# DeepGraphLearning/ultra_torchdrug

Measured on AMD Instinct MI355X. Metric: edges aggregated/sec, FB15k237-shaped 6L x 64d rspmm Bellman-Ford (predict: the reference's 18 rspmm layers per batch as 6 relation-graph + 6 entity-graph launches, tails and heads in one pass), higher is better.
Workload: dtype f32

## Files before the change

ultra_torchdrug_amd/csrc/dense.inc:

```

namespace {

struct LinearParams {
    const float *input;
    const float *weight;
    const float *bias;
    float *out;
    long long rows;
    int relu;
};

template <int K, int N>
__global__ __launch_bounds__(kCbWaves * 64, 1) void linear_kernel(const LinearParams p) {
    static_assert(K == N && (K == 64 || K == 128), "supported shapes: 64x64, 128x128");
    constexpr int kStride = K + 4;
    constexpr int kOutTiles = N / 32;
    extern __shared__ __attribute__((aligned(16))) float dl_lds[];
    float *w_lds = dl_lds;
    const int lane = threadIdx.x & 63;
    const int wl = uniform(threadIdx.x >> 6);
    float *tile = dl_lds + N * kStride + wl * (32 * kStride);
    const int i = lane & 31, h = lane >> 5;
    for (int idx = threadIdx.x; idx < N * (K / 4); idx += kCbWaves * 64) {
        const int r = idx / (K / 4), c = (idx % (K / 4)) * 4;
// ... 334 lines not shown
int launch_linear(const LinearParams &p, int n_cu, hipStream_t stream) {
    constexpr int kStride = K + 4;
    const size_t lds = (size_t)(K * kStride + kCbWaves * 32 * kStride) * sizeof(float);
    const long long n_tiles = (p.rows + 31) / 32;
    long long blocks = (n_tiles + kCbWaves - 1) / kCbWaves;
    if (blocks > n_cu) blocks = n_cu;
    return launch_with_lds(linear_kernel<K, K>, p, (int)blocks, lds, stream, kCbWaves * 64, (int)lds);
}

}

namespace {

constexpr int kProjMaxLayers = 8;
struct ProjectParams {
    const float *relation;
    const float *w1[kProjMaxLayers], *b1[kProjMaxLayers], *w2[kProjMaxLayers], *b2[kProjMaxLayers];
    float *out[kProjMaxLayers];
    long long rows;
    int batch, n_rel, n_layers, blocks_per_layer;
    int repeat;
    long long stride_b, stride_r;
};

__global__ __launch_bounds__(kCbWaves * 64, 1) void project_kernel(const ProjectParams p) {
    constexpr int K = 64, kStride = K + 4;
    extern __shared__ __attribute__((aligned(16))) float pj_lds[];
    float *w1_lds = pj_lds, *w2_lds = pj_lds + K * kStride;
    const int lane = threadIdx.x & 63;
    const int wl = uniform(threadIdx.x >> 6);
    float *tile = pj_lds + 2 * K * kStride + wl * (32 * kStride);
    const int i = lane & 31, h = lane >> 5;
    const int l = blockIdx.x / p.blocks_per_layer, bl = blockIdx.x % p.blocks_per_layer;
    for (int idx = threadIdx.x; idx < K * (K / 4); idx += kCbWaves * 64) {
        const int r = idx / (K / 4), c = (idx % (K / 4)) * 4;
        *reinterpret_cast<f32x4 *>(w1_lds + r * kStride + c) = *reinterpret_cast<const f32x4 *>(p.w1[l] + r * K + c);
        *reinterpret_cast<f32x4 *>(w2_lds + r * kStride + c) = *reinterpret_cast<const f32x4 *>(p.w2[l] + r * K + c);
    }
    __syncthreads();
    const float bias1[2] = {p.b1[l][i], p.b1[l][i + 32]}, bias2[2] = {p.b2[l][i], p.b2[l][i + 32]};
    float *out = p.out[l];
    const long long n_tiles = (p.rows + 31) / 32;
    const long long wave_global = (long long)bl * kCbWaves + wl;
    const long long wave_total = (long long)p.blocks_per_layer * kCbWaves;
    auto gemm = [&](const float *w_lds, const float (&bias)[2], f32x16 (&acc)[2]) {
#pragma unroll
        for (int tt = 0; tt < 2; ++tt)
#pragma unroll
            for (int r = 0; r < 16; ++r) acc[tt][r] = bias[tt];
#pragma unroll
        for (int q = 0; q < K / 8; ++q) {
            const f32x4 av = *reinterpret_cast<const f32x4 *>(tile + i * kStride + (K / 2) * h + 4 * q);
#pragma unroll
            for (int tt = 0; tt < 2; ++tt) {
                const f32x4 wv = *reinterpret_cast<const f32x4 *>(w_lds + (i + 32 * tt) * kStride + (K / 2) * h + 4 * q);
                acc[tt] = __builtin_amdgcn_mfma_f32_32x32x2f32(av.x, wv.x, acc[tt], 0, 0, 0);
                acc[tt] = __builtin_amdgcn_mfma_f32_32x32x2f32(av.y, wv.y, acc[tt], 0, 0, 0);
                acc[tt] = __builtin_amdgcn_mfma_f32_32x32x2f32(av.z, wv.z, acc[tt], 0, 0, 0);
                acc[tt] = __builtin_amdgcn_mfma_f32_32x32x2f32(av.w, wv.w, acc[tt], 0, 0, 0);
            }
        }
        asm volatile("s_waitcnt lgkmcnt(0)" ::: "memory");
    };
    auto spill = [&](const f32x16 (&acc)[2], bool relu) {
#pragma unroll
        for (int tt = 0; tt < 2; ++tt)
#pragma unroll
            for (int r = 0; r < 16; ++r) {
                const int row = (r & 3) + 8 * (r >> 2) + 4 * h;
                float v = acc[tt][r];
                if (relu) v = !(v <= 0.0f) ? v : 0.0f;
                tile[row * kStride + 32 * tt + i] = v;
            }
        asm volatile("s_waitcnt lgkmcnt(0)" ::: "memory");
    };
    for (long long t = wave_global; t < n_tiles; t += wave_total) {
        const long long row0 = t * 32;
        const long long last = p.rows - 1;
#pragma unroll
        for (int q = 0; q < 8; ++q) {
            const int r = 4 * q + (lane >> 4), c = (lane & 15) * 4;
            long long gr = row0 + r;
            gr = gr < last ? gr : last;
            const long long b = gr / p.n_rel, rel = gr - b * p.n_rel;
            *reinterpret_cast<f32x4 *>(tile + r * kStride + c) = *reinterpret_cast<const f32x4 *>(p.relation + b * p.stride_b + rel * p.stride_r + c);
        }
        asm volatile("s_waitcnt vmcnt(0) lgkmcnt(0)" ::: "memory");
        f32x16 acc[2];
        gemm(w1_lds, bias1, acc);
        spill(acc, true);
        gemm(w2_lds, bias2, acc);
        spill(acc, false);
#pragma unroll
        for (int q = 0; q < 8; ++q) {
            const int r = 4 * q + (lane >> 4), c = (lane & 15) * 4;
            const long long gr = row0 + r;
            if (gr < p.rows) {
                const long long b = gr / p.n_rel, rel = gr % p.n_rel;
                const f32x4 v = *reinterpret_cast<const f32x4 *>(tile + r * kStride + c);
                for (int j = 0; j < p.repeat; ++j)
                    *reinterpret_cast<f32x4 *>(out + (rel * ((long long)p.batch * p.repeat) + b + (long long)j * p.batch) * K + c) = v;
            }
        }
        asm volatile("s_waitcnt lgkmcnt(0)" ::: "memory");
    }
}

__global__ __launch_bounds__(256) void filtered_rank_kernel(const float *pred, long long row_stride, long long n_cand,
                                                            const int64_t *target, const int32_t *filt_ptr,
                                                            const int32_t *filt_node, int64_t *rank) {
    __shared__ long long part[4];
    const long long q = blockIdx.x;
    const float *row = pred + q * row_stride;
    const float pos = row[target[q]];
    long long count = 0;
    for (long long c = threadIdx.x; c < n_cand; c += blockDim.x) count += (pos <= row[c]) ? 1 : 0;
    if (filt_ptr != nullptr) {
        const int lo = filt_ptr[q], hi = filt_ptr[q + 1];
        for (int k = lo + (int)threadIdx.x; k < hi; k += (int)blockDim.x) count -= (pos <= row[filt_node[k]]) ? 1 : 0;
    }
#pragma unroll
    for (int off = 32; off > 0; off >>= 1) count += __shfl_down(count, off, 64);
    if ((threadIdx.x & 63) == 0) part[threadIdx.x >> 6] = count;
    __syncthreads();
    if (threadIdx.x == 0) rank[q] = part[0] + part[1] + part[2] + part[3] + 1;
}

}

extern "C" {

// ... 109 lines not shown
```

ultra_torchdrug_amd/csrc/frontier.inc:

```

struct FrontierParams {
    const int32_t *src_ptr;
    const int32_t *dst;
    const int32_t *rel;
    const float *weight;
    const int32_t *fwd_rank;
    const float *relation;
    const int32_t *bnode;
    const float *bvec;
    float *out;
    long long F;
    int piece_len;
    int slices;
    int n_rel;
    int piece_shift;
    const int32_t *run_prefix;
    int32_t *row_list;
    const int32_t *list_offset;
    int list_len;
};

constexpr int kFrontierThreads = 256;
constexpr int kFrontierU = 4;

template <bool UNIT_W>
__global__ __launch_bounds__(kFrontierThreads) void frontier_kernel(const FrontierParams p) {
    const int lane = threadIdx.x & 63;
    const int b = blockIdx.x;
    const long long col = (long long)b * 64 + (lane & 15) * 4;
    const int groups_per_block = kFrontierThreads / 16;
    const int g = blockIdx.y * groups_per_block + (threadIdx.x >> 4);
    const int n_groups = p.slices * groups_per_block;
    const int h = p.bnode[b];
    const qf4 q = *reinterpret_cast<const qf4 *>(p.bvec + col);
    const int lo = p.src_ptr[h], hi = p.src_ptr[h + 1];

    if (g == 0) {
        bool self_loop = false;
        int a = lo, z = hi;
        while (a < z) {
            const int m = (a + z) >> 1;
            if (p.dst[m] < h) a = m + 1; else z = m;
        }
        self_loop = a < hi && p.dst[a] == h;
        if (!self_loop) {
            const qf4 zero = {0.0f, 0.0f, 0.0f, 0.0f};
            *reinterpret_cast<qf4 *>(p.out + (long long)h * p.F + col) = zero + q;
        }
        if (p.row_list != nullptr && (lane & 15) == 0 && p.list_offset[b + 1] - 1 < p.list_len)
            p.row_list[p.list_offset[b + 1] - 1] = self_loop ? -1 : h * (int)(p.F / 64) + b;
    }

// ... 75 lines not shown
        }
#pragma unroll
        for (int u = 0; u < kFrontierU; ++u) {
            if (done) break;
            const int eu = e + u;
            if (eu >= hi) { done = true; break; }
            if (d[u] != cur) {
                if (eu >= end) { done = true; break; }
                close_run();
                cur = d[u];
                run_first = eu;
                cur_piece = -1;
                have_total = false;
            }
            const int piece_of_edge = k[u] / p.piece_len;
            if (piece_of_edge != cur_piece) {
                close_piece();
                cur_piece = piece_of_edge;
                piece_end_rank = (cur_piece + 1) * p.piece_len;
                piece = qf4{0.0f, 0.0f, 0.0f, 0.0f};
            }
            qf4 y = rv[u] * q;
            if constexpr (!UNIT_W) y = w[u] * y;
            piece = piece + y;
        }
        e += kFrontierU;
    }
    close_run();
}

constexpr int kFrontierLdsThreads = 1024;
constexpr int kFrontierLdsSlices = 8;

template <bool UNIT_W>
__global__ __launch_bounds__(kFrontierLdsThreads) void frontier_lds_kernel(const FrontierParams p) {
    extern __shared__ __attribute__((aligned(16))) float fl_msg[];
    const int lane = threadIdx.x & 63;
    const int sub = lane & 15;
    const int n_query = (int)(p.F / 64);
    const int b = blockIdx.x % n_query;
    const int slice = blockIdx.x / n_query;
    const long long col = (long long)b * 64 + sub * 4;
    const int h = p.bnode[b];
    const qf4 q = *reinterpret_cast<const qf4 *>(p.bvec + col);
    {
        const float *rel_b = p.relation + (long long)b * 64;
        const float *q_b = p.bvec + (long long)b * 64;
        for (int i = threadIdx.x; i < p.n_rel * 16; i += kFrontierLdsThreads) {
            const int r = i >> 4, c4 = (i & 15) * 4;
            const qf4 rv = *reinterpret_cast<const qf4 *>(rel_b + (long long)r * p.F + c4);
            const qf4 qq = *reinterpret_cast<const qf4 *>(q_b + c4);
            reinterpret_cast<qf4 *>(fl_msg)[i] = rv * qq;
        }
    }
    __syncthreads();
    const qf4 *msg = reinterpret_cast<const qf4 *>(fl_msg) + sub;

    const int groups_per_block = kFrontierLdsThreads / 16;
    const int g = slice * groups_per_block + (threadIdx.x >> 4);
    const int n_groups = p.slices * groups_per_block;
    const int lo = p.src_ptr[h], hi = p.src_ptr[h + 1];

    const int list_base = p.row_list != nullptr ? p.list_offset[b] : 0;
    if (g == 0) {
        int a = lo, z = hi;
        while (a < z) {
            const int m = (a + z) >> 1;
            if (p.dst[m] < h) a = m + 1; else z = m;
        }
        const bool self_loop = a < hi && p.dst[a] == h;
        if (!self_loop) {
            const qf4 zero = {0.0f, 0.0f, 0.0f, 0.0f};
            *reinterpret_cast<qf4 *>(p.out + (long long)h * p.F + col) = zero + q;
        }
        if (p.row_list != nullptr && sub == 0 && p.list_offset[b + 1] - 1 < p.list_len)
            p.row_list[p.list_offset[b + 1] - 1] = self_loop ? -1 : h * n_query + b;
    }

    const int n = hi - lo;
    if (n <= 0) return;
    const int per = (n + n_groups - 1) / n_groups;
    int e = lo + g * per;
    const int end = min(e + per, hi);
    if (e >= end) return;
    if (e > lo) {
        const int prev = p.dst[e - 1];
        int a = e, step = 1;
        while (a < hi && p.dst[a] == prev) { a += step; step <<= 1; }
        if (a > e) {
            int z = min(a, hi);
            a = a - (step >> 1) + 1;
            while (a < z) {
                const int m = (a + z) >> 1;
                if (p.dst[m] == prev) a = m + 1; else z = m;
            }
        }
        e = a;
    }
    if (e >= end) return;

    int slot = 0;
    if (p.row_list != nullptr) slot = list_base + p.run_prefix[e] - p.run_prefix[lo];
    int cur = p.dst[e];
    int cur_piece = -1;
    bool open = false, have_total = false;
    qf4 total = {0.0f, 0.0f, 0.0f, 0.0f};
    qf4 piece = {0.0f, 0.0f, 0.0f, 0.0f};
    auto close_piece = [&]() {
        if (open) {
            total = have_total ? total + piece : (qf4{0.0f, 0.0f, 0.0f, 0.0f} + piece);
            have_total = true;
        }
    };
    auto close_run = [&](int dest) {
        close_piece();
        qf4 v = total;
        v = v + ((dest == h) ? q : qf4{0.0f, 0.0f, 0.0f, 0.0f});
        *reinterpret_cast<qf4 *>(p.out + (long long)dest * p.F + col) = v;
        if (p.row_list != nullptr) {
            if (sub == 0 && slot < p.list_len) p.row_list[slot] = dest * n_query + b;
            ++slot;
        }
    };
    auto load_ids = [&](int e0, int &d, int &r, int &k, float &w) {
        const int eu = min(e0 + sub, hi - 1);
        d = p.dst[eu];
        r = p.rel[eu];
        k = p.fwd_rank[eu];
        w = 1.0f;
        if constexpr (!UNIT_W) w = p.weight[eu];
    };
    const int bp = (lane & 48) * 4;
    const int grp_shift = (lane >> 4) * 16;
    auto from = [&](int u, int v) -> int { return __builtin_amdgcn_ds_bpermute(bp + 4 * u, v); };

    int nd, nr, nk;
    float nw;
    load_ids(e, nd, nr, nk, nw);
    bool done = false;
    while (!done) {
        const int md = nd, mr = nr, mk = nk;
        const float mw = nw;
        load_ids(e + 16, nd, nr, nk, nw);
        const int mp = p.piece_shift >= 0 ? (mk >> p.piece_shift) : (mk / p.piece_len);
        const int prev_d = __builtin_amdgcn_update_dpp(cur, md, 0x111, 0xf, 0xf, false);
        const int prev_p = __builtin_amdgcn_update_dpp(cur_piece, mp, 0x111, 0xf, 0xf, false);
        const int n_valid = min(16, hi - e);
        const bool starts_run = (md != prev_d) && sub < n_valid;
        const bool starts_piece = (starts_run || mp != prev_p) && sub < n_valid;
        const uint32_t run_bits = (uint32_t)(__builtin_amdgcn_ballot_w64(starts_run) >> grp_shift) & 0xffffu;
        const uint32_t piece_bits = (uint32_t)(__builtin_amdgcn_ballot_w64(starts_piece) >> grp_shift) & 0xffffu;
        const int room = end - e;
        const uint32_t beyond = room >= 16 ? 0u : (room <= 0 ? 0xffffu : (0xffffu << room) & 0xffffu);
        const uint32_t stop_bits = run_bits & beyond;
        const int n_sum = min(n_valid, stop_bits ? __builtin_ctz(stop_bits) : 16);
        done = n_sum < 16;
#pragma unroll
        for (int half = 0; half < 2; ++half) {
            qf4 y[8];
#pragma unroll
            for (int v = 0; v < 8; ++v) {
                const int u = 8 * half + v;
                y[v] = msg[from(u, mr) * 16];
                if constexpr (!UNIT_W) y[v] = __builtin_bit_cast(float, from(u, __builtin_bit_cast(int, mw))) * y[v];
            }
            const uint32_t any = (run_bits | piece_bits) >> (8 * half) & 0xffu;
            if (any == 0u && n_sum >= 8 * half + 8) {
#pragma unroll
                for (int v = 0; v < 8; ++v) piece = piece + y[v];
                continue;
            }
#pragma unroll
            for (int v = 0; v < 8; ++v) {
                const int u = 8 * half + v;
                if (u < n_sum) {
                    if ((run_bits >> u) & 1u) {
                        close_run(u == 0 ? cur : from(u - 1, md));
                        have_total = false;
                        open = false;
                    }
                    if ((piece_bits >> u) & 1u) {
                        close_piece();
                        open = true;
                        piece = qf4{0.0f, 0.0f, 0.0f, 0.0f};
                    }
                    piece = piece + y[v];
                }
            }
        }
        if (n_sum > 0) {
            cur = from(n_sum - 1, md);
            cur_piece = from(n_sum - 1, mp);
        }
        e += 16;
    }
    close_run(cur);
}

constexpr int kSparseMaxQueries = 128;
struct ConstFillParams {
    qf4 *out;
    long long n4;
    const float *bias, *gamma, *beta;
    float eps;
    int relu, shortcut;
    const int32_t *src_ptr, *run_prefix, *bnode;
    int n_query;
    int list_len;
    int32_t *list_offset;
};

__global__ __launch_bounds__(256) void const_fill_kernel(const ConstFillParams p) {
    __shared__ __attribute__((aligned(16))) float c[64];
    __shared__ int slots[kSparseMaxQueries];
    if (threadIdx.x < 64) {
        const int j = threadIdx.x;
        float v = p.bias[j];
        if (p.gamma != nullptr) {
            float s0 = 0.0f, s1 = 0.0f;
            for (int k = 0; k < 32; ++k) { s0 = s0 + p.bias[k]; s1 = s1 + p.bias[32 + k]; }
            const float mean = (s0 + s1) * (1.0f / 64.0f);
            float q0 = 0.0f, q1 = 0.0f;
            for (int k = 0; k < 32; ++k) {
                const float d0 = p.bias[k] - mean, d1 = p.bias[32 + k] - mean;
                q0 = q0 + d0 * d0;
                q1 = q1 + d1 * d1;
            }
            const float var = (q0 + q1) * (1.0f / 64.0f);
            const float inv = 1.0f / sqrtf(var + p.eps);
            v = ((v - mean) * inv) * p.gamma[j] + p.beta[j];
        }
        if (p.relu) v = !(v <= 0.0f) ? v : 0.0f;
        c[j] = p.shortcut ? v + 0.0f : v;
    }
    if (blockIdx.x == 0) {
        if ((int)threadIdx.x < p.n_query) {
            const int h = p.bnode[threadIdx.x];
            const int lo = p.src_ptr[h], hi = p.src_ptr[h + 1];
            slots[threadIdx.x] = (hi > lo ? p.run_prefix[hi - 1] - p.run_prefix[lo] + 1 : 0) + 1;
        }
        __syncthreads();
        if (threadIdx.x == 0) {
            int total = 0;
            for (int b = 0; b < p.n_query; ++b) {
                p.list_offset[b] = total;
                total += slots[b];
            }
            p.list_offset[p.n_query] = total;
        }
    }
    __syncthreads();
    const qf4 *c4 = reinterpret_cast<const qf4 *>(c);
    for (long long i = (long long)blockIdx.x * 256 + threadIdx.x; i < p.n4; i += (long long)gridDim.x * 256) p.out[i] = c4[i & 15];
}

__global__ __launch_bounds__(256) void zero_fill_kernel(qf4 *out, long long n4) {
    const qf4 zero = {0.0f, 0.0f, 0.0f, 0.0f};
    for (long long i = (long long)blockIdx.x * 256 + threadIdx.x; i < n4; i += (long long)gridDim.x * 256) out[i] = zero;
}

struct BoundaryRowsParams {
    const int32_t *src_ptr;
    const int32_t *dst;
    const int32_t *rel;
    const float *weight;
    const float *relation;
    const float *grad;
    const int32_t *bnode;
    float *partial;
    float *d_input;
    long long F;
};

// ... 64 lines not shown
```

ultra_torchdrug_amd/csrc/plan_path.h:

```cpp
#ifndef ULTRA_PLAN_PATH_H
#define ULTRA_PLAN_PATH_H

#include <cstddef>
#include <cstdint>

#include "ultra_rspmm.h"

namespace ultra_detail {

constexpr int kTile = 64;
constexpr int kXcd = 8;
constexpr int kMaxLdsBytes = 156 * 1024;
constexpr int kLdsHeader = 16;
constexpr int kPlanBlock = 1024;
constexpr int kPlanRgBlock = 512;

enum Kind { KIND_FWD = 0, KIND_DX = 1, KIND_DREL = 2 };
enum Family { FAM_DENSE = 0, FAM_ROWGROUP = 1, FAM_QUAD = 2, FAM_PACKED = 3, FAM_GENERAL = 4 };
enum RelMode { REL_L2 = 0, REL_LDS = 1, REL_PART = 2 };
enum ActMode { ACT_NONE = 0, ACT_BITS = 2, ACT_NODE = 3 };
enum UnrollClass { UNROLL_U = 0, UNROLL_UW = 1, UNROLL_UX = 2 };
enum Fixup { FIX_NONE = 0, FIX_PLAIN = 1, FIX_MANY = 2 };

struct Knobs {
    bool force_general = false;
    bool no_x_lds = false;
    bool no_quad = false;
    bool no_rowgroup = false;
    bool wide_groups = false;
    bool no_concurrent_tiles = false;
    bool no_dense = false;
    bool no_dead_words = false;
    bool no_paired = false;
    bool force_paired = false;
    bool score_lds_rows = false;
    bool combine_lds_rows = false;
};

inline Knobs decode_knobs(int mask) {
    Knobs k;
    k.force_general = (mask & 1) != 0;
    k.no_x_lds = (mask & 2) != 0;
    k.no_quad = (mask & 4) != 0;
    k.no_rowgroup = (mask & 8) != 0;
    k.wide_groups = (mask & 16) != 0;
    k.no_concurrent_tiles = (mask & 32) != 0;
    k.no_dense = (mask & 64) != 0;
    k.no_dead_words = (mask & 128) != 0;
    k.no_paired = (mask & 256) != 0;
    k.force_paired = (mask & 512) != 0;
    k.score_lds_rows = (mask & 1024) != 0;
    k.combine_lds_rows = (mask & 2048) != 0;
    return k;
}

inline int gcd_int(int a, int b) {
    while (b) {
        const int t = a % b;
        a = b;
        b = t;
    }
    return a;
}

struct TileGeometry {
    int n_tiles = 0, split = 0, n_slots = 0, blocks_per_label = 0, grid = 0;
};

inline TileGeometry tile_geometry(long long columns, int width, int n_cu) {
    TileGeometry g;
    g.n_tiles = (int)((columns + width - 1) / width);
    g.split = kXcd / gcd_int(g.n_tiles, kXcd);
    g.n_slots = g.n_tiles * g.split;
    g.blocks_per_label = (n_cu + kXcd - 1) / kXcd;
    g.grid = g.blocks_per_label * kXcd;
    return g;
}

struct RowGroupTiling {
    int group = 16;
    int rel_mode = REL_L2;
    int n_rel_lds = 0;
    TileGeometry geo;
    size_t lds = 0;
};
// ... 201 lines not shown
```

ultra_torchdrug_amd/csrc/rspmm_kernels.hip:

```cpp
#include <hip/hip_runtime.h>
#include <type_traits>

#include <algorithm>
#include <cstdint>
#include <cstdlib>
#include <cstring>
#include <mutex>

#include "host_common.h"
#include "launch_record.h"

thread_local int ultra_detail_last_hip_error = 0;

namespace {

using namespace ultra_detail;

#ifndef ULTRA_BLOCK
#define ULTRA_BLOCK 1024
#endif
constexpr int kBlock = ULTRA_BLOCK;
#ifndef ULTRA_UNROLL
#define ULTRA_UNROLL 8
#endif
// ... 1757 lines not shown
    hipStream_t s = static_cast<hipStream_t>(stream);
    hipEvent_t ev_start = g_prof_start, ev_stop = g_prof_stop;
    g_prof_start = g_prof_stop = nullptr;
    if (ev_start != nullptr || ev_stop != nullptr) {
        hipStreamCaptureStatus cs = hipStreamCaptureStatusNone;
        HIP_TRY(hipStreamIsCapturing(s, &cs));
        if (cs != hipStreamCaptureStatusNone) ev_start = ev_stop = nullptr;
    }
    if (ev_start != nullptr) HIP_TRY(hipEventRecord(ev_start, s));
    {
        const long long n4 = (long long)n_dst * F / 4;
        const unsigned blocks = (unsigned)((n4 + 256 * 8 - 1) / (256 * 8) < 4096 ? (n4 + 256 * 8 - 1) / (256 * 8) : 4096);
        hipLaunchKernelGGL(zero_fill_kernel, dim3(blocks ? blocks : 1), dim3(256), 0, s, reinterpret_cast<qf4 *>(out), n4);
        HIP_TRY(hipGetLastError());
    }
    FrontierParams p{};
    p.src_ptr = src_ptr;
    p.dst = by_src->node_a;
    p.rel = by_src->rel;
    p.weight = by_src->weight;
    p.fwd_rank = fwd_rank;
    p.relation = relation;
    p.bnode = boundary_node;
    p.bvec = boundary_value;
    p.out = out;
    p.F = F;
    p.piece_len = (int)by_src->piece_len;
    p.n_rel = (int)n_rel;
    p.piece_shift = -1;
    for (int sh = 0; sh < 31; ++sh)
        if ((1LL << sh) == by_src->piece_len) p.piece_shift = sh;
    const size_t msg_bytes = (size_t)n_rel * kTile * sizeof(float);
    if (!g_knobs.force_general && n_rel > 0 && msg_bytes <= (size_t)kMaxLdsBytes) {
        p.slices = kFrontierLdsSlices;
        const int grid = (int)(F / 64) * p.slices;
        int rc = by_src->weight == nullptr
                     ? launch_with_lds(frontier_lds_kernel<true>, p, grid, msg_bytes, s, kFrontierLdsThreads)
                     : launch_with_lds(frontier_lds_kernel<false>, p, grid, msg_bytes, s, kFrontierLdsThreads);
        if (rc) return rc;
    } else {
        p.slices = 64;
        const dim3 grid((unsigned)(F / 64), (unsigned)p.slices);
        if (by_src->weight == nullptr) hipLaunchKernelGGL(frontier_kernel<true>, grid, dim3(kFrontierThreads), 0, s, p);
        else hipLaunchKernelGGL(frontier_kernel<false>, grid, dim3(kFrontierThreads), 0, s, p);
        HIP_TRY(hipGetLastError());
    }
    if (ev_stop != nullptr) HIP_TRY(hipEventRecord(ev_stop, s));
    return ULTRA_OK;
}

int ultra_first_layer_sparse_supported(int64_t n_dst, int64_t n_rel, int64_t n_query) {
    return n_query > 0 && n_query <= kCbLdsQueries && n_rel > 0 && n_dst > 0 && n_dst * n_query < 0x7fffffffLL;
}

static int first_layer_sparse_impl(const ultra_segments *by_src, const int32_t *src_ptr, const int32_t *fwd_rank,
                                   const int32_t *run_prefix, const float *relation, const int32_t *boundary_node,
                                   const float *boundary_value, int64_t n_query, const float *weight, const float *bias,
                                   const float *ln_weight, const float *ln_bias, float ln_eps, int relu, int shortcut,
                                   float *update, float *out, int32_t *row_list, int64_t row_list_len, int64_t max_runs,
                                   int32_t *list_offset, int64_t n_dst, int64_t n_rel, void *stream) {
    int rc = check_segments(by_src);
    if (rc) return rc;
    if (!ultra_first_layer_sparse_supported(n_dst, n_rel, n_query) || by_src->piece_len <= 0 || max_runs < 0 ||
        max_runs > n_dst || row_list_len < n_query * (max_runs + 1) || row_list_len > 0x7fffffffLL)
        return ULTRA_ERR_BAD_SHAPE;
    if (src_ptr == nullptr || fwd_rank == nullptr || run_prefix == nullptr || relation == nullptr || boundary_node == nullptr ||
        boundary_value == nullptr || weight == nullptr || bias == nullptr || out == nullptr || update == nullptr ||
        row_list == nullptr || list_offset == nullptr)
        return ULTRA_ERR_NULL_POINTER;
    if (ln_weight != nullptr && ln_bias == nullptr) return ULTRA_ERR_NULL_POINTER;
    const long long F = n_query * 64;
    if ((reinterpret_cast<uintptr_t>(out) | reinterpret_cast<uintptr_t>(update) | reinterpret_cast<uintptr_t>(relation) |
         reinterpret_cast<uintptr_t>(boundary_value)) & 15u)
        return ULTRA_ERR_BAD_SHAPE;
    hipStream_t s = static_cast<hipStream_t>(stream);
    DeviceInfo *di = nullptr;
    rc = current_device_info(&di);
    if (rc) return rc;
    CombineParams cp{};
    cp.weight = weight; cp.bias = bias; cp.gamma = ln_weight; cp.beta = ln_bias;
    cp.eps = ln_eps; cp.relu = relu; cp.shortcut = shortcut;
    cp.in_bnode = boundary_node; cp.in_bvec = boundary_value; cp.rpn = (int)n_query;
    const size_t lds_cb = (size_t)(kCbWaves * kCbTileFloats + 128 + n_query * 65) * sizeof(float);
    rc = ensure_lds_attribute(reinterpret_cast<const void *>(combine_kernel<false, 3>), lds_cb);
    if (rc) return rc;
    {
        ConstFillParams fp{};
        fp.out = reinterpret_cast<qf4 *>(out); fp.n4 = (long long)n_dst * F / 4;
        fp.bias = bias; fp.gamma = ln_weight; fp.beta = ln_bias; fp.eps = ln_eps; fp.relu = relu; fp.shortcut = shortcut;
        fp.src_ptr = src_ptr; fp.run_prefix = run_prefix; fp.bnode = boundary_node; fp.n_query = (int)n_query;
        fp.list_offset = list_offset; fp.list_len = (int)row_list_len;
        const unsigned blocks = (unsigned)((fp.n4 + 256 * 8 - 1) / (256 * 8) < 4096 ? (fp.n4 + 256 * 8 - 1) / (256 * 8) : 4096);
        hipLaunchKernelGGL(const_fill_kernel, dim3(blocks ? blocks : 1), dim3(256), 0, s, fp);
        HIP_TRY(hipGetLastError());
    }
    FrontierParams p{};
    p.src_ptr = src_ptr; p.dst = by_src->node_a; p.rel = by_src->rel; p.weight = by_src->weight; p.fwd_rank = fwd_rank;
    p.relation = relation; p.bnode = boundary_node; p.bvec = boundary_value; p.out = update; p.F = F;
    p.piece_len = (int)by_src->piece_len; p.n_rel = (int)n_rel; p.piece_shift = -1;
    for (int sh = 0; sh < 31; ++sh)
        if ((1LL << sh) == by_src->piece_len) p.piece_shift = sh;
    p.run_prefix = run_prefix; p.row_list = row_list; p.list_offset = list_offset; p.list_len = (int)row_list_len;
    const size_t msg_bytes = (size_t)n_rel * kTile * sizeof(float);
    if (!g_knobs.force_general && msg_bytes <= (size_t)kMaxLdsBytes) {
        p.slices = kFrontierLdsSlices;
        const int fgrid = (int)n_query * p.slices;
        rc = by_src->weight == nullptr ? launch_with_lds(frontier_lds_kernel<true>, p, fgrid, msg_bytes, s, kFrontierLdsThreads)
                                       : launch_with_lds(frontier_lds_kernel<false>, p, fgrid, msg_bytes, s, kFrontierLdsThreads);
        if (rc) return rc;
    } else {
        p.slices = 64;
        const dim3 fgrid((unsigned)n_query, (unsigned)p.slices);
        if (by_src->weight == nullptr) hipLaunchKernelGGL(frontier_kernel<true>, fgrid, dim3(kFrontierThreads), 0, s, p);
        else hipLaunchKernelGGL(frontier_kernel<false>, fgrid, dim3(kFrontierThreads), 0, s, p);
        HIP_TRY(hipGetLastError());
    }
    cp.update = update; cp.out = out; cp.rows = n_dst * n_query; cp.row_list = row_list; cp.list_count = list_offset + n_query;
    cp.list_len = (int)row_list_len;
    hipLaunchKernelGGL((combine_kernel<false, 3>), dim3((unsigned)(2 * di->n_cu)), dim3(kCbWaves * 64), lds_cb, s, cp);
    HIP_TRY(hipGetLastError());
    return ULTRA_OK;
}

int ultra_first_layer_sparse_f32(const ultra_segments *by_src, const int32_t *src_ptr, const int32_t *fwd_rank,
                                 const int32_t *run_prefix, const float *relation, const int32_t *boundary_node,
                                 const float *boundary_value, int64_t n_query, const float *weight, const float *bias,
                                 const float *ln_weight, const float *ln_bias, float ln_eps, int relu, int shortcut,
                                 float *out, int32_t *row_list, int64_t row_list_len, int64_t max_runs, int32_t *list_offset,
                                 int64_t n_dst, int64_t n_rel, void *stream) {
    return first_layer_sparse_impl(by_src, src_ptr, fwd_rank, run_prefix, relation, boundary_node, boundary_value, n_query, weight,
                                   bias, ln_weight, ln_bias, ln_eps, relu, shortcut, out, out, row_list, row_list_len, max_runs,
                                   list_offset, n_dst, n_rel, stream);
}

int ultra_first_layer_sparse_train_f32(const ultra_segments *by_src, const int32_t *src_ptr, const int32_t *fwd_rank,
                                       const int32_t *run_prefix, const float *relation, const int32_t *boundary_node,
                                       const float *boundary_value, int64_t n_query, const float *weight, const float *bias,
                                       const float *ln_weight, const float *ln_bias, float ln_eps, int relu, int shortcut,
                                       float *update, float *out, int32_t *row_list, int64_t row_list_len, int64_t max_runs,
                                       int32_t *list_offset, int64_t n_dst, int64_t n_rel, void *stream) {
    if (update == nullptr) return ULTRA_ERR_NULL_POINTER;
// ... 283 lines not shown
```

ultra_torchdrug_amd/functional.py:

```python
import collections
import ctypes
import os

import torch

from . import _lib, _torch_ext
from .relcsr import RelCSR

__all__ = ["generalized_rspmm", "rspmm_forward", "rotate_rspmm", "rotate_rspmm_forward", "rotate_rspmm_backward_weight", "first_layer_forward", "dense_layer_forward", "combine_forward", "combine", "linear_forward", "linear_supported", "score_all_entities", "relation_stack_inputs", "statistics", "bce_adversarial_loss", "candidate_tiles", "candidate_rows", "score_candidates", "hop_distance", "RelCSR"]

_sparse_cache = collections.OrderedDict()
_SPARSE_CACHE_ENTRIES = 4


def accepts(tensor):
    return bool(tensor.is_cuda)


def _ops(sum, mul):
    if sum not in _lib.SUM_OPS:
        raise ValueError("Can't find a rspmm operator for sum=`%s` (expected add, min or max)" % sum)
    if mul not in _lib.MUL_OPS:
        raise ValueError("Can't find a rspmm operator for mul=`%s` (expected mul or add)" % mul)
    return _lib.SUM_OPS[sum], _lib.MUL_OPS[mul]
# ... 213 lines not shown
    dev = relation.device
    src_ptr, fwd_rank = csr.frontier_index
    run_prefix, max_runs = csr.frontier_runs
    out = torch.empty(n_dst, n_query, 64, dtype=torch.float32, device=dev)
    row_list = torch.empty(n_query * (max_runs + 1), dtype=torch.int32, device=dev)
    list_offset = torch.empty(n_query + 1, dtype=torch.int32, device=dev)
    head = (csr.by_src.pointer, src_ptr, fwd_rank, run_prefix, relation, b_node, b_value, n_query)
    tail = (out, row_list, row_list.numel(), int(max_runs), list_offset, n_dst, n_rel)
    return dev, head, tail, out, row_list, list_offset


def first_layer_forward(csr, relation, boundary, weight, bias, ln_weight=None, ln_bias=None, ln_eps=1e-5, relu=True,
                        shortcut=False, want_list=False):
    if not SPARSE_FIRST_LAYER:
        return None
    b_node, b_value = boundary
    n_dst, n_src, n_rel = csr.shape
    n_query = b_node.shape[0]
    lib = _lib.load()
    if (n_dst != n_src or n_dst * n_query < SPARSE_FIRST_LAYER_MIN_ROWS
            or not lib.ultra_first_layer_sparse_supported(n_dst, n_rel, n_query)
            or csr.frontier_runs[1] + 1 > SPARSE_FIRST_LAYER_MAX_LIST * n_dst):
        return None
    F = n_query * 64
    b_value = b_value.contiguous()
    tensors = [relation, b_value, weight, bias] + ([ln_weight, ln_bias] if ln_weight is not None else [])
    if (relation.dim() != 2 or tuple(relation.shape) != (n_rel, F) or tuple(b_value.shape) != (n_query, 64) or b_node.dtype != torch.int32
            or not b_node.is_contiguous() or tuple(weight.shape) != (64, 128)
            or _not_fp32_on(relation.device, tensors)
            or b_node.device != relation.device or csr.device != relation.device):
        raise RuntimeError("first_layer_forward: relation fp32 (%d, %d), boundary (int32 (Q,), fp32 (Q, 64)), a (64, 128) weight, "
                           "all on one HIP device" % (n_rel, F))
    dev, head, tail, out, row_list, list_offset = _first_layer_arguments(csr, relation, b_node, b_value)
    _launch(dev, "ultra_first_layer_sparse_f32", *head, *_epilogue(weight, bias, ln_weight, ln_bias, ln_eps, relu, shortcut), *tail)
    if want_list:
        return out, row_list, list_offset[n_query:]
    return out


SPARSE_FIRST_LAYER_TRAIN = _env_bool("ULTRA_SPARSE_FIRST_LAYER_TRAIN", True)
SPARSE_FIRST_LAYER_TRAIN_MAX_FRACTION = _env_float("ULTRA_SPARSE_FIRST_LAYER_TRAIN_MAX_FRACTION", 0.2)


def first_layer_train_forward(csr, relation, boundary, weight, bias, ln_weight=None, ln_bias=None, ln_eps=1e-5, relu=True,
                              shortcut=False):
    if not SPARSE_FIRST_LAYER_TRAIN:
        return None
    b_node, b_value = boundary
    n_dst, n_src, n_rel = csr.shape
    n_query = b_node.shape[0]
    lib = _lib.load()
    if (n_dst != n_src or n_dst * n_query < SPARSE_FIRST_LAYER_MIN_ROWS or n_dst * n_query > (1 << 24) - 64
            or not lib.ultra_first_layer_sparse_supported(n_dst, n_rel, n_query)
            or csr.frontier_fraction > SPARSE_FIRST_LAYER_TRAIN_MAX_FRACTION
            or csr.frontier_runs[1] + 1 > SPARSE_FIRST_LAYER_MAX_LIST * n_dst
            or n_query * (csr.frontier_runs[1] + 1) * 5 * 256 > SPARSE_FIRST_LAYER_TRAIN_MAX_BYTES):
        return None
    F = n_query * 64
    b_value = b_value.contiguous()
    if (tuple(relation.shape) != (n_rel, F) or tuple(b_value.shape) != (n_query, 64) or b_node.dtype != torch.int32
            or not b_node.is_contiguous() or tuple(weight.shape) != (64, 128)):
        return None
    update = torch.empty(n_dst, n_query, 64, dtype=torch.float32, device=relation.device)
    dev, head, tail, out, row_list, list_offset = _first_layer_arguments(csr, relation, b_node, b_value)
    _launch(dev, "ultra_first_layer_sparse_train_f32", *head, *_epilogue(weight, bias, ln_weight, ln_bias, ln_eps, relu, shortcut),
            update, *tail)
    return update, out, row_list, list_offset[n_query:]
# ... 1304 lines not shown
```

Baseline: 46.95 billion.

## Fuse constant fill into frontier kernel and prefetch projection input rows

Folds the first-layer constant-fill pass (bias/LN constant row, per-query list offsets) into the LDS frontier kernel, so one launch replaces two and the fill overlaps with the sparse walk. The inference path now calls the train entry point with a separate update buffer so the fused path is taken. In the relation projection kernel, input rows for the first tile are loaded before the weight staging, and row indices are computed once per tile in 32-bit arithmetic. The fused kernel needs extra LDS and has every block recompute the list prefix sums, and a knob restores the previous path.

```diff
diff --git a/ultra_torchdrug_amd/csrc/dense.inc b/ultra_torchdrug_amd/csrc/dense.inc
--- a/ultra_torchdrug_amd/csrc/dense.inc
+++ b/ultra_torchdrug_amd/csrc/dense.inc
@@ -390,17 +390,42 @@
     float *tile = pj_lds + 2 * K * kStride + wl * (32 * kStride);
     const int i = lane & 31, h = lane >> 5;
     const int l = blockIdx.x / p.blocks_per_layer, bl = blockIdx.x % p.blocks_per_layer;
+    const long long n_tiles = (p.rows + 31) / 32;
+    const long long wave_global = (long long)bl * kCbWaves + wl;
+    const long long wave_total = (long long)p.blocks_per_layer * kCbWaves;
+    int row_b[8], row_rel[8], live = 0;
+    auto rows_of = [&](long long t) {
+        const long long row0 = t * 32;
+        const int b0 = (int)(row0 / p.n_rel);
+        const unsigned rel0 = (unsigned)(row0 - (long long)b0 * p.n_rel);
+        const long long left = p.rows - row0;
+        live = left < 32 ? (int)left : 32;
+#pragma unroll
+        for (int q = 0; q < 8; ++q) {
+            const int r = 4 * q + (lane >> 4);
+            const unsigned x = rel0 + (unsigned)(r < live ? r : live - 1);
+            row_b[q] = b0 + (int)(x / (unsigned)p.n_rel);
+            row_rel[q] = (int)(x % (unsigned)p.n_rel);
+        }
+    };
+    f32x4 in[8];
+    auto request = [&]() {
+#pragma unroll
+        for (int q = 0; q < 8; ++q)
+            in[q] = *reinterpret_cast<const f32x4 *>(p.relation + row_b[q] * p.stride_b + row_rel[q] * p.stride_r + (lane & 15) * 4);
+    };
+    if (wave_global < n_tiles) {
+        rows_of(wave_global);
+        request();
+    }
+    const float bias1[2] = {p.b1[l][i], p.b1[l][i + 32]}, bias2[2] = {p.b2[l][i], p.b2[l][i + 32]};
     for (int idx = threadIdx.x; idx < K * (K / 4); idx += kCbWaves * 64) {
         const int r = idx / (K / 4), c = (idx % (K / 4)) * 4;
         *reinterpret_cast<f32x4 *>(w1_lds + r * kStride + c) = *reinterpret_cast<const f32x4 *>(p.w1[l] + r * K + c);
         *reinterpret_cast<f32x4 *>(w2_lds + r * kStride + c) = *reinterpret_cast<const f32x4 *>(p.w2[l] + r * K + c);
     }
     __syncthreads();
-    const float bias1[2] = {p.b1[l][i], p.b1[l][i + 32]}, bias2[2] = {p.b2[l][i], p.b2[l][i + 32]};
     float *out = p.out[l];
-    const long long n_tiles = (p.rows + 31) / 32;
-    const long long wave_global = (long long)bl * kCbWaves + wl;
-    const long long wave_total = (long long)p.blocks_per_layer * kCbWaves;
     auto gemm = [&](const float *w_lds, const float (&bias)[2], f32x16 (&acc)[2]) {
 #pragma unroll
         for (int tt = 0; tt < 2; ++tt)
@@ -433,15 +458,14 @@
         asm volatile("s_waitcnt lgkmcnt(0)" ::: "memory");
     };
     for (long long t = wave_global; t < n_tiles; t += wave_total) {
-        const long long row0 = t * 32;
-        const long long last = p.rows - 1;
+        if (t != wave_global) {
+            rows_of(t);
+            request();
+        }
 #pragma unroll
         for (int q = 0; q < 8; ++q) {
             const int r = 4 * q + (lane >> 4), c = (lane & 15) * 4;
-            long long gr = row0 + r;
-            gr = gr < last ? gr : last;
-            const long long b = gr / p.n_rel, rel = gr - b * p.n_rel;
-            *reinterpret_cast<f32x4 *>(tile + r * kStride + c) = *reinterpret_cast<const f32x4 *>(p.relation + b * p.stride_b + rel * p.stride_r + c);
+            *reinterpret_cast<f32x4 *>(tile + r * kStride + c) = in[q];
         }
         asm volatile("s_waitcnt vmcnt(0) lgkmcnt(0)" ::: "memory");
         f32x16 acc[2];
@@ -452,9 +476,8 @@
 #pragma unroll
         for (int q = 0; q < 8; ++q) {
             const int r = 4 * q + (lane >> 4), c = (lane & 15) * 4;
-            const long long gr = row0 + r;
-            if (gr < p.rows) {
-                const long long b = gr / p.n_rel, rel = gr % p.n_rel;
+            if (r < live) {
+                const long long b = row_b[q], rel = row_rel[q];
                 const f32x4 v = *reinterpret_cast<const f32x4 *>(tile + r * kStride + c);
                 for (int j = 0; j < p.repeat; ++j)
                     *reinterpret_cast<f32x4 *>(out + (rel * ((long long)p.batch * p.repeat) + b + (long long)j * p.batch) * K + c) = v;
diff --git a/ultra_torchdrug_amd/csrc/frontier.inc b/ultra_torchdrug_amd/csrc/frontier.inc
--- a/ultra_torchdrug_amd/csrc/frontier.inc
+++ b/ultra_torchdrug_amd/csrc/frontier.inc
@@ -1,3 +1,42 @@
+
+constexpr int kSparseMaxQueries = 128;
+struct ConstFillParams {
+    qf4 *out;
+    long long n4;
+    const float *bias, *gamma, *beta;
+    float eps;
+    int relu, shortcut;
+    const int32_t *src_ptr, *run_prefix, *bnode;
+    int n_query;
+    int list_len;
+    int32_t *list_offset;
+};
+
+__device__ __forceinline__ float const_row_value(const ConstFillParams &p, int j) {
+    float v = p.bias[j];
+    if (p.gamma != nullptr) {
+        float s0 = 0.0f, s1 = 0.0f;
+        for (int k = 0; k < 32; ++k) { s0 = s0 + p.bias[k]; s1 = s1 + p.bias[32 + k]; }
+        const float mean = (s0 + s1) * (1.0f / 64.0f);
+        float q0 = 0.0f, q1 = 0.0f;
+        for (int k = 0; k < 32; ++k) {
+            const float d0 = p.bias[k] - mean, d1 = p.bias[32 + k] - mean;
+            q0 = q0 + d0 * d0;
+            q1 = q1 + d1 * d1;
+        }
+        const float var = (q0 + q1) * (1.0f / 64.0f);
+        const float inv = 1.0f / sqrtf(var + p.eps);
+        v = ((v - mean) * inv) * p.gamma[j] + p.beta[j];
+    }
+    if (p.relu) v = !(v <= 0.0f) ? v : 0.0f;
+    return p.shortcut ? v + 0.0f : v;
+}
+
+__device__ __forceinline__ int query_slots(const ConstFillParams &p, int b) {
+    const int h = p.bnode[b];
+    const int lo = p.src_ptr[h], hi = p.src_ptr[h + 1];
+    return (hi > lo ? p.run_prefix[hi - 1] - p.run_prefix[lo] + 1 : 0) + 1;
+}
 
 struct FrontierParams {
     const int32_t *src_ptr;
@@ -18,6 +57,7 @@
     int32_t *row_list;
     const int32_t *list_offset;
     int list_len;
+    ConstFillParams fill;
 };
 
 constexpr int kFrontierThreads = 256;
@@ -159,10 +199,15 @@
 constexpr int kFrontierLdsThreads = 1024;
 constexpr int kFrontierLdsSlices = 8;
 
-template <bool UNIT_W>
+constexpr int kFrontierLdsFillBytes = 256 + 16;
+
+template <bool UNIT_W, bool FILL>
 __global__ __launch_bounds__(kFrontierLdsThreads) void frontier_lds_kernel(const FrontierParams p) {
     extern __shared__ __attribute__((aligned(16))) float fl_msg[];
+    float *fl_const = fl_msg + (long long)p.n_rel * 64;
+    int *fl_list = reinterpret_cast<int *>(fl_const + 64);
     const int lane = threadIdx.x & 63;
+    const int wave = uniform(threadIdx.x >> 6);
     const int sub = lane & 15;
     const int n_query = (int)(p.F / 64);
     const int b = blockIdx.x % n_query;
@@ -170,6 +215,33 @@
     const long long col = (long long)b * 64 + sub * 4;
     const int h = p.bnode[b];
     const qf4 q = *reinterpret_cast<const qf4 *>(p.bvec + col);
+    const int lo = p.src_ptr[h], hi = p.src_ptr[h + 1];
+    if constexpr (FILL) {
+        if (wave == 15) fl_const[lane] = const_row_value(p.fill, lane);
+        if (wave == 14) {
+            int before = 0, mine = 0, all = 0;
+#pragma unroll
+            for (int half = 0; half < kSparseMaxQueries / 64; ++half) {
+                const int qi = lane + 64 * half;
+                const int s = qi < n_query ? query_slots(p.fill, qi) : 0;
+                before += qi < b ? s : 0;
+                mine += qi == b ? s : 0;
+                all += s;
+            }
+#pragma unroll
+            for (int off = 32; off > 0; off >>= 1) {
+                before += __shfl_xor(before, off, 64);
+                mine += __shfl_xor(mine, off, 64);
+                all += __shfl_xor(all, off, 64);
+            }
+            if (lane == 0) {
+                fl_list[0] = before;
+                fl_list[1] = before + mine;
+                if (slice == 0) p.fill.list_offset[b] = before;
+                if (blockIdx.x == 0) p.fill.list_offset[n_query] = all;
+            }
+        }
+    }
     {
         const float *rel_b = p.relation + (long long)b * 64;
         const float *q_b = p.bvec + (long long)b * 64;
@@ -183,12 +255,18 @@
     __syncthreads();
     const qf4 *msg = reinterpret_cast<const qf4 *>(fl_msg) + sub;
 
+    int list_base = 0, list_next = 0;
+    if (p.row_list != nullptr) {
+        if constexpr (FILL) {
+            list_base = fl_list[0];
+            list_next = fl_list[1];
+        } else {
+            list_base = p.list_offset[b];
+        }
+    }
     const int groups_per_block = kFrontierLdsThreads / 16;
     const int g = slice * groups_per_block + (threadIdx.x >> 4);
     const int n_groups = p.slices * groups_per_block;
-    const int lo = p.src_ptr[h], hi = p.src_ptr[h + 1];
-
-    const int list_base = p.row_list != nullptr ? p.list_offset[b] : 0;
     if (g == 0) {
         int a = lo, z = hi;
         while (a < z) {
@@ -200,17 +278,18 @@
             const qf4 zero = {0.0f, 0.0f, 0.0f, 0.0f};
             *reinterpret_cast<qf4 *>(p.out + (long long)h * p.F + col) = zero + q;
         }
-        if (p.row_list != nullptr && sub == 0 && p.list_offset[b + 1] - 1 < p.list_len)
-            p.row_list[p.list_offset[b + 1] - 1] = self_loop ? -1 : h * n_query + b;
+        if (p.row_list != nullptr) {
+            if constexpr (!FILL) list_next = p.list_offset[b + 1];
+            if (sub == 0 && list_next - 1 < p.list_len) p.row_list[list_next - 1] = self_loop ? -1 : h * n_query + b;
+        }
     }
 
     const int n = hi - lo;
-    if (n <= 0) return;
-    const int per = (n + n_groups - 1) / n_groups;
+    const int per = n > 0 ? (n + n_groups - 1) / n_groups : 0;
     int e = lo + g * per;
     const int end = min(e + per, hi);
-    if (e >= end) return;
-    if (e > lo) {
+    bool walk = n > 0 && e < end;
+    if (walk && e > lo) {
         const int prev = p.dst[e - 1];
         int a = e, step = 1;
         while (a < hi && p.dst[a] == prev) { a += step; step <<= 1; }
@@ -224,31 +303,7 @@
         }
         e = a;
     }
-    if (e >= end) return;
-
-    int slot = 0;
-    if (p.row_list != nullptr) slot = list_base + p.run_prefix[e] - p.run_prefix[lo];
-    int cur = p.dst[e];
-    int cur_piece = -1;
-    bool open = false, have_total = false;
-    qf4 total = {0.0f, 0.0f, 0.0f, 0.0f};
-    qf4 piece = {0.0f, 0.0f, 0.0f, 0.0f};
-    auto close_piece = [&]() {
-        if (open) {
-            total = have_total ? total + piece : (qf4{0.0f, 0.0f, 0.0f, 0.0f} + piece);
-            have_total = true;
-        }
-    };
-    auto close_run = [&](int dest) {
-        close_piece();
-        qf4 v = total;
-        v = v + ((dest == h) ? q : qf4{0.0f, 0.0f, 0.0f, 0.0f});
-        *reinterpret_cast<qf4 *>(p.out + (long long)dest * p.F + col) = v;
-        if (p.row_list != nullptr) {
-            if (sub == 0 && slot < p.list_len) p.row_list[slot] = dest * n_query + b;
-            ++slot;
-        }
-    };
+    walk = walk && e < end;
     auto load_ids = [&](int e0, int &d, int &r, int &k, float &w) {
         const int eu = min(e0 + sub, hi - 1);
         d = p.dst[eu];
@@ -257,115 +312,123 @@
         w = 1.0f;
         if constexpr (!UNIT_W) w = p.weight[eu];
     };
-    const int bp = (lane & 48) * 4;
-    const int grp_shift = (lane >> 4) * 16;
-    auto from = [&](int u, int v) -> int { return __builtin_amdgcn_ds_bpermute(bp + 4 * u, v); };
-
-    int nd, nr, nk;
-    float nw;
-    load_ids(e, nd, nr, nk, nw);
-    bool done = false;
-    while (!done) {
-        const int md = nd, mr = nr, mk = nk;
-        const float mw = nw;
-        load_ids(e + 16, nd, nr, nk, nw);
-        const int mp = p.piece_shift >= 0 ? (mk >> p.piece_shift) : (mk / p.piece_len);
-        const int prev_d = __builtin_amdgcn_update_dpp(cur, md, 0x111, 0xf, 0xf, false);
-        const int prev_p = __builtin_amdgcn_update_dpp(cur_piece, mp, 0x111, 0xf, 0xf, false);
-        const int n_valid = min(16, hi - e);
-        const bool starts_run = (md != prev_d) && sub < n_valid;
-        const bool starts_piece = (starts_run || mp != prev_p) && sub < n_valid;
-        const uint32_t run_bits = (uint32_t)(__builtin_amdgcn_ballot_w64(starts_run) >> grp_shift) & 0xffffu;
-        const uint32_t piece_bits = (uint32_t)(__builtin_amdgcn_ballot_w64(starts_piece) >> grp_shift) & 0xffffu;
-        const int room = end - e;
-        const uint32_t beyond = room >= 16 ? 0u : (room <= 0 ? 0xffffu : (0xffffu << room) & 0xffffu);
-        const uint32_t stop_bits = run_bits & beyond;
-        const int n_sum = min(n_valid, stop_bits ? __builtin_ctz(stop_bits) : 16);
-        done = n_sum < 16;
-#pragma unroll
-        for (int half = 0; half < 2; ++half) {
-            qf4 y[8];
-#pragma unroll
-            for (int v = 0; v < 8; ++v) {
-                const int u = 8 * half + v;
-                y[v] = msg[from(u, mr) * 16];
-                if constexpr (!UNIT_W) y[v] = __builtin_bit_cast(float, from(u, __builtin_bit_cast(int, mw))) * y[v];
-            }
-            const uint32_t any = (run_bits | piece_bits) >> (8 * half) & 0xffu;
-            if (any == 0u && n_sum >= 8 * half + 8) {
-#pragma unroll
-                for (int v = 0; v < 8; ++v) piece = piece + y[v];
-                continue;
-            }
-#pragma unroll
-            for (int v = 0; v < 8; ++v) {
-                const int u = 8 * half + v;
-                if (u < n_sum) {
-                    if ((run_bits >> u) & 1u) {
-                        close_run(u == 0 ? cur : from(u - 1, md));
-                        have_total = false;
-                        open = false;
+    if (walk) {
+        int slot = 0;
+        if (p.row_list != nullptr) slot = list_base + p.run_prefix[e] - p.run_prefix[lo];
+        int cur = p.dst[e];
+        int cur_piece = -1;
+        bool open = false, have_total = false;
+        qf4 total = {0.0f, 0.0f, 0.0f, 0.0f};
+        qf4 piece = {0.0f, 0.0f, 0.0f, 0.0f};
+        auto close_piece = [&]() {
+            if (open) {
+                total = have_total ? total + piece : (qf4{0.0f, 0.0f, 0.0f, 0.0f} + piece);
+                have_total = true;
+            }
+        };
+        auto close_run = [&](int dest) {
+            close_piece();
+            qf4 v = total;
+            v = v + ((dest == h) ? q : qf4{0.0f, 0.0f, 0.0f, 0.0f});
+            *reinterpret_cast<qf4 *>(p.out + (long long)dest * p.F + col) = v;
+            if (p.row_list != nullptr) {
+                if (sub == 0 && slot < p.list_len) p.row_list[slot] = dest * n_query + b;
+                ++slot;
+            }
+        };
+        const int bp = (lane & 48) * 4;
+        const int grp_shift = (lane >> 4) * 16;
+        auto from = [&](int u, int v) -> int { return __builtin_amdgcn_ds_bpermute(bp + 4 * u, v); };
+
+        int nd, nr, nk;
+        float nw;
+        load_ids(e, nd, nr, nk, nw);
+        bool done = false;
+        while (!done) {
+            const int md = nd, mr = nr, mk = nk;
+            const float mw = nw;
+            load_ids(e + 16, nd, nr, nk, nw);
+            const int mp = p.piece_shift >= 0 ? (mk >> p.piece_shift) : (mk / p.piece_len);
+            const int prev_d = __builtin_amdgcn_update_dpp(cur, md, 0x111, 0xf, 0xf, false);
+            const int prev_p = __builtin_amdgcn_update_dpp(cur_piece, mp, 0x111, 0xf, 0xf, false);
+            const int n_valid = min(16, hi - e);
+            const bool starts_run = (md != prev_d) && sub < n_valid;
+            const bool starts_piece = (starts_run || mp != prev_p) && sub < n_valid;
+            const uint32_t run_bits = (uint32_t)(__builtin_amdgcn_ballot_w64(starts_run) >> grp_shift) & 0xffffu;
+            const uint32_t piece_bits = (uint32_t)(__builtin_amdgcn_ballot_w64(starts_piece) >> grp_shift) & 0xffffu;
+            const int room = end - e;
+            const uint32_t beyond = room >= 16 ? 0u : (room <= 0 ? 0xffffu : (0xffffu << room) & 0xffffu);
+            const uint32_t stop_bits = run_bits & beyond;
+            const int n_sum = min(n_valid, stop_bits ? __builtin_ctz(stop_bits) : 16);
+            done = n_sum < 16;
+#pragma unroll
+            for (int half = 0; half < 2; ++half) {
+                qf4 y[8];
+#pragma unroll
+                for (int v = 0; v < 8; ++v) {
+                    const int u = 8 * half + v;
+                    y[v] = msg[from(u, mr) * 16];
+                    if constexpr (!UNIT_W) y[v] = __builtin_bit_cast(float, from(u, __builtin_bit_cast(int, mw))) * y[v];
+                }
+                const uint32_t any = (run_bits | piece_bits) >> (8 * half) & 0xffu;
+                if (any == 0u && n_sum >= 8 * half + 8) {
+#pragma unroll
+                    for (int v = 0; v < 8; ++v) piece = piece + y[v];
+                    continue;
+                }
+#pragma unroll
+                for (int v = 0; v < 8; ++v) {
+                    const int u = 8 * half + v;
+                    if (u < n_sum) {
+                        if ((run_bits >> u) & 1u) {
+                            close_run(u == 0 ? cur : from(u - 1, md));
+                            have_total = false;
+                            open = false;
+                        }
+                        if ((piece_bits >> u) & 1u) {
+                            close_piece();
+                            open = true;
+                            piece = qf4{0.0f, 0.0f, 0.0f, 0.0f};
+                        }
+                        piece = piece + y[v];
                     }
-                    if ((piece_bits >> u) & 1u) {
-                        close_piece();
-                        open = true;
-                        piece = qf4{0.0f, 0.0f, 0.0f, 0.0f};
-                    }
-                    piece = piece + y[v];
                 }
             }
-        }
-        if (n_sum > 0) {
-            cur = from(n_sum - 1, md);
-            cur_piece = from(n_sum - 1, mp);
-        }
-        e += 16;
-    }
-    close_run(cur);
-}
-
-constexpr int kSparseMaxQueries = 128;
-struct ConstFillParams {
-    qf4 *out;
-    long long n4;
-    const float *bias, *gamma, *beta;
-    float eps;
-    int relu, shortcut;
-    const int32_t *src_ptr, *run_prefix, *bnode;
-    int n_query;
-    int list_len;
-    int32_t *list_offset;
-};
+            if (n_sum > 0) {
+                cur = from(n_sum - 1, md);
+                cur_piece = from(n_sum - 1, mp);
+            }
+            e += 16;
+        }
+        close_run(cur);
+    }
+
+    if constexpr (FILL) {
+        const long long n_waves = (long long)gridDim.x * (kFrontierLdsThreads / 64);
+        const long long w = (long long)blockIdx.x * (kFrontierLdsThreads / 64) + wave;
+        const long long share = p.fill.n4 / n_waves;
+        const long long first = w * share;
+        const long long last = w == n_waves - 1 ? p.fill.n4 : first + share;
+        const qf4 cv = reinterpret_cast<const qf4 *>(fl_const)[(first + lane) & 15];
+        for (long long i = first + lane; i < last; i += 64) p.fill.out[i] = cv;
+    }
+}
+
+template <bool FILL>
+int launch_frontier_lds(FrontierParams &p, int n_query, size_t lds, hipStream_t stream) {
+    p.slices = kFrontierLdsSlices;
+    const int grid = n_query * p.slices;
+    return with_bool(p.weight == nullptr, [&](auto unit) {
+        return launch_with_lds(frontier_lds_kernel<decltype(unit)::value, FILL>, p, grid, lds, stream, kFrontierLdsThreads);
+    });
+}
 
 __global__ __launch_bounds__(256) void const_fill_kernel(const ConstFillParams p) {
     __shared__ __attribute__((aligned(16))) float c[64];
     __shared__ int slots[kSparseMaxQueries];
-    if (threadIdx.x < 64) {
-        const int j = threadIdx.x;
-        float v = p.bias[j];
-        if (p.gamma != nullptr) {
-            float s0 = 0.0f, s1 = 0.0f;
-            for (int k = 0; k < 32; ++k) { s0 = s0 + p.bias[k]; s1 = s1 + p.bias[32 + k]; }
-            const float mean = (s0 + s1) * (1.0f / 64.0f);
-            float q0 = 0.0f, q1 = 0.0f;
-            for (int k = 0; k < 32; ++k) {
-                const float d0 = p.bias[k] - mean, d1 = p.bias[32 + k] - mean;
-                q0 = q0 + d0 * d0;
-                q1 = q1 + d1 * d1;
-            }
-            const float var = (q0 + q1) * (1.0f / 64.0f);
-            const float inv = 1.0f / sqrtf(var + p.eps);
-            v = ((v - mean) * inv) * p.gamma[j] + p.beta[j];
-        }
-        if (p.relu) v = !(v <= 0.0f) ? v : 0.0f;
-        c[j] = p.shortcut ? v + 0.0f : v;
-    }
+    if (threadIdx.x < 64) c[threadIdx.x] = const_row_value(p, (int)threadIdx.x);
     if (blockIdx.x == 0) {
-        if ((int)threadIdx.x < p.n_query) {
-            const int h = p.bnode[threadIdx.x];
-            const int lo = p.src_ptr[h], hi = p.src_ptr[h + 1];
-            slots[threadIdx.x] = (hi > lo ? p.run_prefix[hi - 1] - p.run_prefix[lo] + 1 : 0) + 1;
-        }
+        if ((int)threadIdx.x < p.n_query) slots[threadIdx.x] = query_slots(p, (int)threadIdx.x);
         __syncthreads();
         if (threadIdx.x == 0) {
             int total = 0;
diff --git a/ultra_torchdrug_amd/csrc/plan_path.h b/ultra_torchdrug_amd/csrc/plan_path.h
--- a/ultra_torchdrug_amd/csrc/plan_path.h
+++ b/ultra_torchdrug_amd/csrc/plan_path.h
@@ -35,6 +35,7 @@
     bool force_paired = false;
     bool score_lds_rows = false;
     bool combine_lds_rows = false;
+    bool former_first_layer = false;
 };
 
 inline Knobs decode_knobs(int mask) {
@@ -51,6 +52,7 @@
     k.force_paired = (mask & 512) != 0;
     k.score_lds_rows = (mask & 1024) != 0;
     k.combine_lds_rows = (mask & 2048) != 0;
+    k.former_first_layer = (mask & 4096) != 0;
     return k;
 }
 
diff --git a/ultra_torchdrug_amd/csrc/rspmm_kernels.hip b/ultra_torchdrug_amd/csrc/rspmm_kernels.hip
--- a/ultra_torchdrug_amd/csrc/rspmm_kernels.hip
+++ b/ultra_torchdrug_amd/csrc/rspmm_kernels.hip
@@ -1813,11 +1813,7 @@
         if ((1LL << sh) == by_src->piece_len) p.piece_shift = sh;
     const size_t msg_bytes = (size_t)n_rel * kTile * sizeof(float);
     if (!g_knobs.force_general && n_rel > 0 && msg_bytes <= (size_t)kMaxLdsBytes) {
-        p.slices = kFrontierLdsSlices;
-        const int grid = (int)(F / 64) * p.slices;
-        int rc = by_src->weight == nullptr
-                     ? launch_with_lds(frontier_lds_kernel<true>, p, grid, msg_bytes, s, kFrontierLdsThreads)
-                     : launch_with_lds(frontier_lds_kernel<false>, p, grid, msg_bytes, s, kFrontierLdsThreads);
+        int rc = launch_frontier_lds<false>(p, (int)(F / 64), msg_bytes, s);
         if (rc) return rc;
     } else {
         p.slices = 64;
@@ -1865,12 +1861,16 @@
     const size_t lds_cb = (size_t)(kCbWaves * kCbTileFloats + 128 + n_query * 65) * sizeof(float);
     rc = ensure_lds_attribute(reinterpret_cast<const void *>(combine_kernel<false, 3>), lds_cb);
     if (rc) return rc;
-    {
-        ConstFillParams fp{};
-        fp.out = reinterpret_cast<qf4 *>(out); fp.n4 = (long long)n_dst * F / 4;
-        fp.bias = bias; fp.gamma = ln_weight; fp.beta = ln_bias; fp.eps = ln_eps; fp.relu = relu; fp.shortcut = shortcut;
-        fp.src_ptr = src_ptr; fp.run_prefix = run_prefix; fp.bnode = boundary_node; fp.n_query = (int)n_query;
-        fp.list_offset = list_offset; fp.list_len = (int)row_list_len;
+    const size_t msg_bytes = (size_t)n_rel * kTile * sizeof(float);
+    const bool lds_form = !g_knobs.force_general && msg_bytes <= (size_t)kMaxLdsBytes;
+    const bool fill_in_frontier = lds_form && update != out && !g_knobs.former_first_layer &&
+                                  msg_bytes + kFrontierLdsFillBytes <= (size_t)kMaxLdsBytes;
+    ConstFillParams fp{};
+    fp.out = reinterpret_cast<qf4 *>(out); fp.n4 = (long long)n_dst * F / 4;
+    fp.bias = bias; fp.gamma = ln_weight; fp.beta = ln_bias; fp.eps = ln_eps; fp.relu = relu; fp.shortcut = shortcut;
+    fp.src_ptr = src_ptr; fp.run_prefix = run_prefix; fp.bnode = boundary_node; fp.n_query = (int)n_query;
+    fp.list_offset = list_offset; fp.list_len = (int)row_list_len;
+    if (!fill_in_frontier) {
         const unsigned blocks = (unsigned)((fp.n4 + 256 * 8 - 1) / (256 * 8) < 4096 ? (fp.n4 + 256 * 8 - 1) / (256 * 8) : 4096);
         hipLaunchKernelGGL(const_fill_kernel, dim3(blocks ? blocks : 1), dim3(256), 0, s, fp);
         HIP_TRY(hipGetLastError());
@@ -1882,12 +1882,12 @@
     for (int sh = 0; sh < 31; ++sh)
         if ((1LL << sh) == by_src->piece_len) p.piece_shift = sh;
     p.run_prefix = run_prefix; p.row_list = row_list; p.list_offset = list_offset; p.list_len = (int)row_list_len;
-    const size_t msg_bytes = (size_t)n_rel * kTile * sizeof(float);
-    if (!g_knobs.force_general && msg_bytes <= (size_t)kMaxLdsBytes) {
-        p.slices = kFrontierLdsSlices;
-        const int fgrid = (int)n_query * p.slices;
-        rc = by_src->weight == nullptr ? launch_with_lds(frontier_lds_kernel<true>, p, fgrid, msg_bytes, s, kFrontierLdsThreads)
-                                       : launch_with_lds(frontier_lds_kernel<false>, p, fgrid, msg_bytes, s, kFrontierLdsThreads);
+    if (fill_in_frontier) {
+        p.fill = fp;
+        rc = launch_frontier_lds<true>(p, (int)n_query, msg_bytes + kFrontierLdsFillBytes, s);
+        if (rc) return rc;
+    } else if (lds_form) {
+        rc = launch_frontier_lds<false>(p, (int)n_query, msg_bytes, s);
         if (rc) return rc;
     } else {
         p.slices = 64;
diff --git a/ultra_torchdrug_amd/functional.py b/ultra_torchdrug_amd/functional.py
--- a/ultra_torchdrug_amd/functional.py
+++ b/ultra_torchdrug_amd/functional.py
@@ -269,7 +269,9 @@
         raise RuntimeError("first_layer_forward: relation fp32 (%d, %d), boundary (int32 (Q,), fp32 (Q, 64)), a (64, 128) weight, "
                            "all on one HIP device" % (n_rel, F))
     dev, head, tail, out, row_list, list_offset = _first_layer_arguments(csr, relation, b_node, b_value)
-    _launch(dev, "ultra_first_layer_sparse_f32", *head, *_epilogue(weight, bias, ln_weight, ln_bias, ln_eps, relu, shortcut), *tail)
+    update = torch.empty_like(out)
+    _launch(dev, "ultra_first_layer_sparse_train_f32", *head, *_epilogue(weight, bias, ln_weight, ln_bias, ln_eps, relu, shortcut),
+            update, *tail)
     if want_list:
         return out, row_list, list_offset[n_query:]
     return out
```

Measured after the change: 47.31 billion (median of 6 runs). No clear change (+0.8%).
